# fema-ffrd/gpras

Hardware: AMD Instinct MI355X
Metric: gp_fits_per_sec (higher is better)
Workload: dtype f64; 1 GPU; BASELINE configs[1] as the many-independent-cells workload: exact GP N=4096 d=8 RBF, fit F1 = kernel build + blocked fp64-MFMA Cholesky + alpha + LML, per cell; cells = y columns of one training set with per-cell hyperparameters (the reference's per-mode models); n_train=4096, d=8, kernel=RBF, collective=none (one process), launcher=single process

## Files before the change

### gpras_amd/_lib.py

```python

from __future__ import annotations

import ctypes as C
from pathlib import Path

import numpy as np

import os

LIB_PATH = Path(os.environ["GPRX_LIBRARY"]) if os.environ.get("GPRX_LIBRARY") else Path(__file__).resolve().parent / "libgprx.so"

GPRX_OK, GPRX_EINVAL, GPRX_ENOTPD, GPRX_EHIP, GPRX_ENOMEM, GPRX_ESTATE, GPRX_ERCCL, GPRX_ENOCONV = range(8)
UNIQUE_ID_BYTES = 128
TRAIN_VARIANCE, TRAIN_LENGTHSCALE, TRAIN_NOISE, TRAIN_Z = 1, 2, 4, 8
GEMM_C_LOWER, GEMM_A_LOWER, GEMM_A_UPPER, GEMM_B_LOWER, GEMM_B_UPPER = 1, 2, 4, 8, 16
REDUCE_LOGDET_QUAD, REDUCE_COL, REDUCE_ROWSQ_FINAL, REDUCE_ROW = range(4)

DISTANCE_FORMS = {"difference": 0, "expanded": 1}
KERNEL_IDS = {"RBF": 0, "Matern12": 1, "Matern32": 2, "Matern52": 3, "Exponential": 4}


class GprxLibraryError(RuntimeError):
    """libgprx.so is missing or unusable."""

# ... 120 lines not shown
    "gprx_hms_last_error": (C.c_char_p, [_vp]),
    "gprx_api": (C.c_int, [C.c_int, _vp, _i64, _vp, _i64, _i64, _vp]),
    "gprx_spline_eval": (C.c_int, [C.c_int, _vp, C.c_int, _vp, _vp, _i64, _vp]),
    "gprx_ps_create": (C.c_int, [C.c_int, _i64, _vp, _vp, _i64, _vp, _vp, C.c_int, _vp, _vp, C.c_int, _vp, C.POINTER(_vp)]),
    "gprx_ps_destroy": (C.c_int, [_vp]),
    "gprx_ps_last_error": (C.c_char_p, [_vp]),
    "gprx_ps_set_weights": (C.c_int, [_vp, _vp]),
    "gprx_ps_fit_centerline": (C.c_int, [_vp, _vp, _vp, _vp, _vp, _vp, _i64, _vp]),
    "gprx_ps_timings": (C.c_int, [_vp, _dp]),
    "gprx_ps_rating": (C.c_int, [_vp, _vp, _vp, _i64, _vp, _vp]),
    "gprx_ps_set_boundaries": (C.c_int, [_vp, _vp, _vp, _i64]),
    "gprx_ps_centerline": (C.c_int, [_vp, _vp]),
    "gprx_ps_gather": (C.c_int, [_vp, _vp, _i64, _vp]),
    "gprx_ps_surface": (C.c_int, [_vp, _vp, _vp]),
    "gprx_ps_surface_dev": (C.c_int, [_vp, _i64, _i64, _vp, _i64, _vp, _i64]),
    "gprx_ps_synchronize": (C.c_int, [_vp]),
    "gprx_pca_slab_rows": (C.c_int, [_vp, C.POINTER(_i64)]),
    "gprx_rs_create": (C.c_int, [C.c_int, _i64, _i64, C.c_int, _vp, _vp, _vp, C.POINTER(_vp)]),
    "gprx_rs_destroy": (C.c_int, [_vp]),
    "gprx_rs_last_error": (C.c_char_p, [_vp]),
    "gprx_rs_apply": (C.c_int, [_vp, _vp, _vp, _i64, _vp]),
    "gprx_rs_apply_dev": (C.c_int, [_vp, _i64, _vp, _i64, _vp, _vp, _i64]),
    "gprx_rs_synchronize": (C.c_int, [_vp]),
    "gprx_rs_timings": (C.c_int, [_vp, _dp]),
    "gprx_al_create": (C.c_int, [C.c_int, C.POINTER(_vp)]),
    "gprx_al_destroy": (C.c_int, [_vp]),
    "gprx_al_last_error": (C.c_char_p, [_vp]),
    "gprx_al_synchronize": (C.c_int, [_vp]),
    "gprx_al_cutoff_dev": (C.c_int, [_vp, C.c_int, _vp, _vp, _vp, _i64, C.c_double, C.POINTER(_i64), C.POINTER(_i64), C.POINTER(_i64), _vp]),
    "gprx_al_cutoff": (C.c_int, [_vp, _vp, _i64, _i64, C.c_double, C.POINTER(_i64), C.POINTER(_i64), C.POINTER(_i64), _vp]),
    "gprx_al_clip_dev": (C.c_int, [_vp, _vp, _i64, _i64, _i64, _i64, _vp, _i64]),
    "gprx_al_timings": (C.c_int, [_vp, _dp]),
    "gprx_dg_create": (C.c_int, [C.c_int, C.POINTER(_vp)]),
    "gprx_dg_destroy": (C.c_int, [_vp]),
    "gprx_dg_last_error": (C.c_char_p, [_vp]),
    "gprx_dg_synchronize": (C.c_int, [_vp]),
    "gprx_dg_sort_u64_dev": (C.c_int, [_vp, _vp, _i64, _vp]),
    "gprx_dg_sort_abs_residual_dev": (C.c_int, [_vp, _vp, _vp, _i64, _vp]),
    "gprx_dg_sort_info": (C.c_int, [_vp, _ip, _dp]),
    "gprx_dg_gather_dev": (C.c_int, [_vp, _vp, _i64, _vp, _i64, _vp]),
    "gprx_dg_scatter_summary_dev": (C.c_int, [_vp, _vp, _vp, _i64, _vp]),
    "gprx_dg_detect_dev": (C.c_int, [_vp, _vp, _vp, _i64, _i64, _vp, _vp, _i64, C.c_double, C.c_int, _vp, C.POINTER(_i64)]),
    "gprx_ev_create": (C.c_int, [C.c_int, _i64, _i64, _i64, _vp, _vp, _vp, _vp, _vp, C.POINTER(_vp)]),
    "gprx_ev_create_empty": (C.c_int, [C.c_int, C.POINTER(_vp)]),
    "gprx_ev_destroy": (C.c_int, [_vp]),
    "gprx_ev_last_error": (C.c_char_p, [_vp]),
    "gprx_ev_synchronize": (C.c_int, [_vp]),
    "gprx_ev_maxima": (C.c_int, [_vp, _vp, _vp, _vp]),
    "gprx_ev_return_periods": (C.c_int, [_vp, _i64, _vp, _vp, _vp]),
    "gprx_ev_rp_eval": (C.c_int, [_vp, C.c_int, _vp, _i64, _vp]),
    "gprx_ev_cov": (C.c_int, [_vp, C.c_int, _vp, _vp]),
    "gprx_ev_eigh": (C.c_int, [_vp, _vp, _vp, _ip]),
    "gprx_ev_scores": (C.c_int, [_vp, C.c_int, C.c_int, _vp]),
    "gprx_ev_standardise": (C.c_int, [_vp, _vp]),
    "gprx_ev_farthest": (C.c_int, [_vp, _vp, _i64, C.c_int, _vp, _i64, _i64, _vp, _vp]),
    "gprx_ev_timings": (C.c_int, [_vp, _dp]),
    "gprx_metrics": (C.c_int, [C.c_int, _vp, _vp, _vp, _i64, _i64, C.c_int, C.c_double, _vp, _vp, _vp, C.POINTER(C.c_uint64)]),
    "gprx_metrics_dev": (C.c_int, [C.c_int, _vp, _vp, _vp, _i64, _i64, C.c_int, C.c_double, _vp, _vp, _vp, C.POINTER(C.c_uint64)]),
    "gprx_kmeans_pp": (C.c_int, [C.c_int, _vp, _i64, C.c_int, _vp, C.c_int, C.c_int, _i64, _vp, _vp]),
    "gprx_kmeans_lloyd": (C.c_int, [C.c_int, _vp, _i64, C.c_int, _vp, C.c_int, C.c_double, C.c_int, _vp, _ip, _ip]),
    "gprx_gather_rows": (C.c_int, [C.c_int, _vp, _i64, _i64, _vp, _vp]),
    "gprx_kmat": (C.c_int, [C.c_int, C.c_int, _vp, _i64, _vp, _i64, C.c_int, _vp, C.c_double, C.c_double, _vp, _i64, _i64, _i64, C.c_int]),
    "gprx_gemm": (C.c_int, [C.c_int, C.c_int, C.c_int, _i64, _i64, _i64, C.c_double, _vp, _i64, _vp, _i64, C.c_double, _vp, _i64, C.c_int, C.c_int]),
    "gprx_potrf": (C.c_int, [C.c_int, _vp, _i64, _i64, _i64, _vp, _ip]),
    "gprx_gemm_batched": (C.c_int, [C.c_int, C.c_int, C.c_int, _i64, _i64, _i64, C.c_double, _vp, _i64, _vp, _i64, C.c_double, _vp, _i64, C.c_int, C.c_int,
                                    C.c_int, _i64, _i64, _i64, C.c_int, _i64, _i64, _i64, _vp, C.c_int, _vp, _i64]),
    "gprx_gemm_splitk": (C.c_int, [C.c_int, C.c_int, C.c_int, _i64, _i64, _i64, C.c_double, _vp, _i64, _vp, _i64, C.c_double, _vp, _i64, _vp, C.c_int,
                                   C.c_int, _i64, _i64, _i64, _i64, _vp, C.c_int]),
    "gprx_trsv_lower": (C.c_int, [C.c_int, _vp, _i64, _vp, _vp, _i64, C.c_int, C.c_int, _i64, _vp]),
    "gprx_potrf_batched": (C.c_int, [C.c_int, _vp, _i64, _i64, _i64, _vp, _vp, _vp, C.c_int, _i64, C.c_int, C.c_int, C.c_int, C.c_int, C.c_int, _ip]),
    "gprx_trsm_lower_left": (C.c_int, [C.c_int, _vp, _i64, _vp, _vp, _i64, _i64, _i64, C.c_int, _i64, _vp]),
    "gprx_trtri_lower": (C.c_int, [C.c_int, _vp, _i64, _vp, _vp, _i64, _vp, _i64, _i64, C.c_int, _i64, _i64, C.c_int]),
    "gprx_transpose_inplace": (C.c_int, [C.c_int, _vp, _i64, _i64, C.c_int, _i64]),
    "gprx_alpha_from_inverse": (C.c_int, [C.c_int, _vp, _i64, _vp, _vp, _vp, _i64, C.c_int, _i64, _i64, _i64]),
    "gprx_reduce_probe": (C.c_int, [C.c_int, C.c_int, _vp, _i64, _vp, _i64, _i64, C.c_double, C.c_double, C.c_int, _vp, C.c_int, _vp, C.c_int, _i64, _i64,
                                    _i64, _i64, _vp, _vp, C.c_int]),
    "gprx_set_tuning": (C.c_int, [C.c_char_p, C.c_int]),
    "gprx_set_handle_tuning": (C.c_int, [_vp, C.c_char_p, C.c_int]),
    "gprx_mfma_f64_peak": (C.c_int, [C.c_int, _dp]),
    "gprx_exp_probe": (C.c_int, [C.c_int, C.c_int, _vp, _i64, _vp]),
}

TUNING_KEYS = (
    "outer_block", "update_tile", "no_lookahead", "split_panel", "dag", "rhs_vector", "rows_pair", "cell_kernel", "poison_workspace", "predict_path",
    "sgpr_fused", "sgpr_resident", "wait_handover_us", "sgpr_groups_from", "loeo_blocked_potrf",
    "held_general",
    "pcafit_rowsplit",
)
PCAFIT_ROUTES = ("gram", "covariance")

_lib = None


def load():
    global _lib
    if _lib is not None:
        return _lib
    if not LIB_PATH.exists():
        raise GprxLibraryError(
            f"{LIB_PATH} not found: build it with `python -c 'import __graft_entry__ as g; g.build()'` "
            "(hipcc --offload-arch=gfx950).  gpras_amd has no CPU fallback."
        )
    try:
        lib = C.CDLL(str(LIB_PATH))
    except OSError as exc:
        raise GprxLibraryError(f"cannot load {LIB_PATH}: {exc}") from exc
    for name, (res, args) in PROTOTYPES.items():
        try:
            fn = getattr(lib, name)
        except AttributeError as exc:
            raise GprxLibraryError(f"{LIB_PATH} does not export {name}") from exc
        fn.restype = res
        fn.argtypes = args
    _lib = lib
    return lib


def last_error(handle=None) -> str:
    msg = load().gprx_last_error(handle)
    return msg.decode() if msg else ""


def check(rc: int, handle=None) -> None:
    if rc == GPRX_OK:
        return
    msg = last_error(handle)
    if rc == GPRX_EINVAL:
        raise ValueError(msg)
    if rc == GPRX_ENOTPD:
        raise np.linalg.LinAlgError(msg)
    if rc == GPRX_ENOCONV:
        raise np.linalg.LinAlgError(msg)
    if rc == GPRX_ENOMEM:
        raise MemoryError(msg)
    raise RuntimeError(f"libgprx error {rc}: {msg}")


def as_f64(a) -> np.ndarray:
    return np.ascontiguousarray(a, dtype=np.float64)


def ptr(a: np.ndarray):
    return _vp(a.ctypes.data)


class DeviceBuffer:

    def __init__(self, nbytes: int, device: int = 0):
        self.device = device
        self.nbytes = int(nbytes)
        p = _vp()
        check(load().gprx_dev_malloc(device, self.nbytes, C.byref(p)))
        self.ptr = p

    @classmethod
    def from_array(cls, a, device: int = 0) -> "DeviceBuffer":
        a = as_f64(a)
        buf = cls(a.nbytes, device)
        check(load().gprx_memcpy_h2d(device, buf.ptr, ptr(a), a.nbytes))
        return buf

    def to_array(self, shape) -> np.ndarray:
        out = np.empty(shape, dtype=np.float64)
        assert out.nbytes <= self.nbytes
        check(load().gprx_memcpy_d2h(self.device, ptr(out), self.ptr, out.nbytes))
        return out

# ... 14 lines not shown
```

### gpras_amd/csrc/gprx.hip

```cpp
#include "abi_common.h"

#include <algorithm>
#include <chrono>
#include <cmath>
#include <cstdio>
#include <cstdlib>
#include <cstring>
#include <limits>
#include <map>
#include <mutex>
#include <string>
#include <thread>
#include <vector>

#include "gemm_f64.h"
#include "gprx_common.h"
#include "grad.h"
#include "kmat.h"
#include "potrf.h"
#include "potrf_cell.h"
#include "potrf_dag.h"
#include "sgpr.h"
#include "sgpr_asm.h"
#include "sgpr_fused.h"
// ... 593 lines not shown

int gprx_gemm_splitk(int device, int ta, int tb, int64_t m, int64_t n, int64_t k, double alpha, const double* a_dev, int64_t lda,
                     const double* b_dev, int64_t ldb, double beta, double* c_dev, int64_t ldc, double* ws_dev, int kchunk, int cells,
                     int64_t cell_a, int64_t cell_b, int64_t cell_c, int64_t ws_cell, const double* alpha_tab_dev, int alpha_stride) {
  return guarded(nullptr, [&]() -> int {
    if (const char* why = gemm_probe_invalid(ta, tb, m, n, k, a_dev, lda, b_dev, ldb, c_dev, ldc)) return fail(nullptr, GPRX_EINVAL, why);
    if (!ws_dev || off16(ws_dev)) return fail(nullptr, GPRX_EINVAL, "workspace must be given, 16-byte aligned");
    if (kchunk <= 0 || kchunk % GEMM_BK) return fail(nullptr, GPRX_EINVAL, "kchunk must be a positive multiple of 16");
    if (cells < 1 || alpha_stride < 0) return fail(nullptr, GPRX_EINVAL, "cells must be positive");
    if (odd(cell_a) || odd(cell_b) || odd(cell_c) || odd(ws_cell) || cell_a < 0 || cell_b < 0 || cell_c < 0)
      return fail(nullptr, GPRX_EINVAL, "cell strides must be even");
    if (cells > 1 && ws_cell < (k + kchunk - 1) / kchunk * m * n) return fail(nullptr, GPRX_EINVAL, "ws_cell shorter than the slabs of one cell");
    HIPCHK(nullptr, hipSetDevice(device));
    HIPCHK(nullptr, launch_gemm_splitk(util_stream(), ta, tb, (int)m, (int)n, (int)k, alpha, a_dev, lda, b_dev, ldb, beta, c_dev, ldc, ws_dev, kchunk,
                                       cells, cell_a, cell_b, cell_c, ws_cell, alpha_tab_dev, alpha_stride));
    HIPCHK(nullptr, hipStreamSynchronize(util_stream()));
    return GPRX_OK;
  });
}

int gprx_trsv_lower(int device, const double* l_dev, int64_t lda, const double* inv_diag_dev, double* b_dev, int64_t np, int transpose,
                    int batch, int64_t cs, double* work_dev) {
  return guarded(nullptr, [&]() -> int {
    if (const char* why = solve_probe_invalid(l_dev, lda, inv_diag_dev, np, batch, cs)) return fail(nullptr, GPRX_EINVAL, why);
    if (!b_dev || (work_dev && (!transpose || batch != 1))) return fail(nullptr, GPRX_EINVAL, "work is for the transposed solve of one system");
    HIPCHK(nullptr, hipSetDevice(device));
    HIPCHK(nullptr, trsv_lower(util_stream(), l_dev, lda, inv_diag_dev, b_dev, (int)np, transpose != 0, batch, cs, work_dev));
    HIPCHK(nullptr, hipStreamSynchronize(util_stream()));
    return GPRX_OK;
  });
}

int gprx_trsm_lower_left(int device, const double* l_dev, int64_t lda, const double* inv_diag_dev, double* b_dev, int64_t ldb, int64_t n,
                         int64_t ncols, int cells, int64_t cs, const double* src_dev) {
  return guarded(nullptr, [&]() -> int {
    if (const char* why = solve_probe_invalid(l_dev, lda, inv_diag_dev, n, cells, cs)) return fail(nullptr, GPRX_EINVAL, why);
    if (!b_dev || off16(b_dev) || (src_dev && off16(src_dev))) return fail(nullptr, GPRX_EINVAL, "right-hand side must be given, 16-byte aligned");
    if (ncols <= 0 || ncols > (1 << 30) || ldb < ncols || odd(ldb)) return fail(nullptr, GPRX_EINVAL, "ldb must be even and at least ncols");
    if (src_dev && n != NB) return fail(nullptr, GPRX_EINVAL, "src is for n == 64 only");
    HIPCHK(nullptr, hipSetDevice(device));
    HIPCHK(nullptr, trsm_lower_left(util_stream(), l_dev, lda, inv_diag_dev, b_dev, ldb, (int)n, (int)ncols, cells, cs, src_dev));
    HIPCHK(nullptr, hipStreamSynchronize(util_stream()));
    return GPRX_OK;
  });
}

int gprx_trtri_lower(int device, const double* l_dev, int64_t lda, const double* inv_diag_dev, double* x_dev, int64_t ldx, double* t_dev,
                     int64_t ldt, int64_t np, int cells, int64_t cs_l, int64_t cs_x, int tile) {
  return guarded(nullptr, [&]() -> int {
    if (const char* why = solve_probe_invalid(l_dev, lda, inv_diag_dev, np, cells, cs_l)) return fail(nullptr, GPRX_EINVAL, why);
    if (!x_dev || !t_dev || off16(x_dev) || off16(t_dev)) return fail(nullptr, GPRX_EINVAL, "X and T must be given, 16-byte aligned");
    if (ldx < np || ldt < np || odd(ldx) || odd(ldt) || odd(cs_x) || cs_x < 0) return fail(nullptr, GPRX_EINVAL, "ldx, ldt, cs_x must be even, rows at least np");
    if (tile != 0 && tile != 64 && tile != 128) return fail(nullptr, GPRX_EINVAL, "tile must be 0, 64 or 128");
    HIPCHK(nullptr, hipSetDevice(device));
    HIPCHK(nullptr, trtri_lower(util_stream(), l_dev, lda, inv_diag_dev, x_dev, ldx, t_dev, ldt, (int)np, cells, cs_l, cs_x, tile));
    HIPCHK(nullptr, hipStreamSynchronize(util_stream()));
    return GPRX_OK;
  });
}

int gprx_potrf_batched(int device, double* a_dev, int64_t lda, int64_t np, int64_t extra, double* inv_diag_dev, double* stage_dev,
                       double* yvec_dev, int batch, int64_t cs, int route, int outer_block, int update_tile, int lookahead, int col_base,
                       int* info_host) {
  return guarded(nullptr, [&]() -> int {
    if (!a_dev || !inv_diag_dev || !stage_dev || !info_host) return fail(nullptr, GPRX_EINVAL, "null argument");
    if (np <= 0 || np % NB) return fail(nullptr, GPRX_EINVAL, "np must be a positive multiple of 64");
    if (extra < 0 || np > (1 << 30) || extra > (1 << 30)) return fail(nullptr, GPRX_EINVAL, "extra must not be negative, np and extra at most 2^30");
    if (lda < np || odd(lda) || odd(cs) || cs < 0) return fail(nullptr, GPRX_EINVAL, "lda and cs must be even, lda at least np");
    if (batch > 1 && cs < lda * (np + extra)) return fail(nullptr, GPRX_EINVAL, "cs shorter than one cell's matrix: the cells would overlap");
    if (off16(a_dev) || off16(inv_diag_dev) || off16(stage_dev) || (yvec_dev && off16(yvec_dev)))
      return fail(nullptr, GPRX_EINVAL, "operands must be 16-byte aligned");
    if (batch < 1 || route < 0 || route > 2 || col_base < 0) return fail(nullptr, GPRX_EINVAL, "batch must be positive, route 0, 1 or 2");
    if (yvec_dev && (route != 1 || batch == 1 || extra != 0))
      return fail(nullptr, GPRX_EINVAL, "the vector right-hand side is the split panel's, for batched cells without right-hand-side rows");
    if (route == 2 && extra % NB) return fail(nullptr, GPRX_EINVAL, "the cell kernel takes right-hand-side rows in tiles of 64");
    if (lookahead != 0 && (lookahead != 1 || batch > 1 || route == 2)) return fail(nullptr, GPRX_EINVAL, "look-ahead is for one matrix on routes 0 and 1");
    if (outer_block < 0 || outer_block % NB || (update_tile != 0 && update_tile != 64 && update_tile != 128))
      return fail(nullptr, GPRX_EINVAL, "outer_block must be a multiple of 64, update_tile 0, 64 or 128");
    PotrfTuning tune;
    tune.outer_block = outer_block;
    tune.update_tile = update_tile;
    tune.split_panel = route == 1 ? 1 : -1;
    tune.rows_pair = potrf_tuning().rows_pair;
    HIPCHK(nullptr, hipSetDevice(device));
    hipStream_t st = util_stream();
    int* dinfo = nullptr;
    HIPCHK(nullptr, hipMalloc((void**)&dinfo, sizeof(int) * batch));
    hipError_t e = memset_sync(dinfo, 0, sizeof(int) * batch);
    PotrfStreams ps;
    if (e == hipSuccess && lookahead) e = ps.init();
    if (e == hipSuccess)
      e = route == 2 ? potrf_cells(st, a_dev, lda, (int)np, (int)extra, inv_diag_dev, dinfo, batch, cs, 1, col_base)
                     : potrf_lower(st, a_dev, lda, (int)np, (int)extra, inv_diag_dev, dinfo, stage_dev, nullptr, lookahead ? &ps : nullptr, batch, cs, 1,
                                   &tune, col_base, yvec_dev);
    hipError_t e2 = hipStreamSynchronize(st);
    if (ps.aux && e2 == hipSuccess) e2 = hipStreamSynchronize(ps.aux);
    ps.destroy();
    if (e == hipSuccess && e2 == hipSuccess) e2 = copy_sync(info_host, dinfo, sizeof(int) * batch, hipMemcpyDeviceToHost);
    hipFree(dinfo);
    HIPCHK(nullptr, e);
    HIPCHK(nullptr, e2);
    for (int c = 0; c < batch; ++c)
      if (info_host[c]) return fail(nullptr, GPRX_ENOTPD, "matrix not positive definite");
    return GPRX_OK;
  });
}

int gprx_transpose_inplace(int device, double* x_dev, int64_t ld, int64_t n, int cells, int64_t cs) {
  return guarded(nullptr, [&]() -> int {
    if (!x_dev || off16(x_dev)) return fail(nullptr, GPRX_EINVAL, "X must be given, 16-byte aligned");
    if (n <= 0 || n % 64 || n > (1 << 30) || ld < n || odd(ld) || cells < 1 || odd(cs) || cs < 0)
      return fail(nullptr, GPRX_EINVAL, "n must be a positive multiple of 64, ld and cs even");
    HIPCHK(nullptr, hipSetDevice(device));
    HIPCHK(nullptr, transpose_inplace(util_stream(), x_dev, ld, (int)n, cells, cs));
    HIPCHK(nullptr, hipStreamSynchronize(util_stream()));
    return GPRX_OK;
  });
}

int gprx_alpha_from_inverse(int device, const double* x_dev, int64_t ldx, const double* beta_dev, double* part_dev, double* alpha_dev, int64_t np,
                            int cells, int64_t cs_x, int64_t cs_b, int64_t cs_a) {
  return guarded(nullptr, [&]() -> int {
    if (!x_dev || !beta_dev || !part_dev || !alpha_dev) return fail(nullptr, GPRX_EINVAL, "null argument");
    if (np <= 0 || np % NB || np > (1 << 30) || ldx < np || cells < 1 || cs_x < 0 || cs_b < 0 || cs_a < 0)
      return fail(nullptr, GPRX_EINVAL, "np must be a positive multiple of 64");
    HIPCHK(nullptr, hipSetDevice(device));
    HIPCHK(nullptr, alpha_from_inverse(util_stream(), x_dev, ldx, beta_dev, part_dev, alpha_dev, (int)np, cells, cs_x, cs_b, cs_a));
    HIPCHK(nullptr, hipStreamSynchronize(util_stream()));
    return GPRX_OK;
  });
}

int gprx_reduce_probe(int device, int op, const double* m_dev, int64_t ldm, const double* w_dev, int64_t nrows, int64_t ncols, double base,
                      double scale, int accumulate, double* partial_dev, int rows_per_chunk, double* out_dev, int cells, int64_t m_cell,
                      int64_t w_cell, int64_t p_cell, int64_t out_cell, const double* base_tab_dev, const double* base_tab2_dev, int base_stride) {
  return guarded(nullptr, [&]() -> int {
    if (!m_dev || !out_dev) return fail(nullptr, GPRX_EINVAL, "null argument");
    if (nrows <= 0 || ncols <= 0 || nrows > (1 << 30) || ncols > (1 << 30) || cells < 1) return fail(nullptr, GPRX_EINVAL, "sizes must be positive");
    if (m_cell < 0 || w_cell < 0 || p_cell < 0 || out_cell < 0 || base_stride < 0) return fail(nullptr, GPRX_EINVAL, "negative stride");
    hipStream_t st = nullptr;
    switch (op) {
      case GPRX_REDUCE_LOGDET_QUAD:
        if (ldm < nrows || ncols != nrows || out_cell > (1 << 30)) return fail(nullptr, GPRX_EINVAL, "logdet_quad: square matrix, ldm at least its order");
        HIPCHK(nullptr, hipSetDevice(device));
        st = util_stream();
        hipLaunchKernelGGL(logdet_quad_kernel, dim3(cells), dim3(256), 0, st, m_dev, ldm, w_dev, (int)nrows, out_dev, m_cell, (int)out_cell);
        break;
      case GPRX_REDUCE_COL: {
        if (ldm < ncols || !partial_dev || rows_per_chunk < 1) return fail(nullptr, GPRX_EINVAL, "colreduce: partial and rows_per_chunk needed");
        const int nchunks = (int)((nrows + rows_per_chunk - 1) / rows_per_chunk);
        if (cells > 1 && p_cell < (int64_t)nchunks * ncols) return fail(nullptr, GPRX_EINVAL, "colreduce: p_cell shorter than the partial sums of one cell");
        HIPCHK(nullptr, hipSetDevice(device));
        st = util_stream();
        hipLaunchKernelGGL(colreduce_partial, dim3((unsigned)((ncols + 255) / 256), nchunks, cells), dim3(256), 0, st, m_dev, ldm, w_dev, (int)nrows,
                           (int)ncols, rows_per_chunk, partial_dev, m_cell, w_cell, p_cell);
        hipLaunchKernelGGL(colreduce_final, dim3((unsigned)((ncols + 255) / 256), cells), dim3(256), 0, st, (const double*)partial_dev, nchunks,
                           (int)ncols, base, scale, accumulate, out_dev, p_cell, out_cell, base_tab_dev, base_tab2_dev, base_stride);
        break;
      }
      case GPRX_REDUCE_ROWSQ_FINAL:
        if (ldm < nrows || cells != 1) return fail(nullptr, GPRX_EINVAL, "rowsq_final: one cell, ldm at least nrows");
        HIPCHK(nullptr, hipSetDevice(device));
        st = util_stream();
        hipLaunchKernelGGL(rowsq_final_kernel, dim3((unsigned)((nrows + 255) / 256)), dim3(256), 0, st, m_dev, (int)ncols, ldm, (int)nrows, base, out_dev);
        break;
      case GPRX_REDUCE_ROW:
// ... 5 lines not shown
                           out_dev);
        break;
      default:
        return fail(nullptr, GPRX_EINVAL, "unknown reduction");
    }
    HIPCHK(nullptr, hipGetLastError());
    HIPCHK(nullptr, hipStreamSynchronize(st));
    return GPRX_OK;
  });
}

extern "C" int gprx_dag_stamps(gprx_handle h, unsigned long long* out, int max_words, int* T, int* grid) {
  if (!h || !h->dag.stamps) return 0;
  const int n = (int)std::min<size_t>(h->dag.stamp_words, (size_t)max_words);
  hipStreamSynchronize(h->stream);
  copy_sync(out, h->dag.stamps, sizeof(unsigned long long) * n, hipMemcpyDeviceToHost);
  if (T) *T = h->dag.T;
  if (grid) *grid = h->dag.grid;
  return n;
}

#ifdef GPRX_CHAIN_STAMPS
extern "C" int gprx_chain_stamps(unsigned long long* out16) {
  hipMemcpyFromSymbol(out16, HIP_SYMBOL(gprx::g_chain_stamps), sizeof(unsigned long long) * 16);
  return 0;
}
#endif

#ifdef GPRX_PANEL_ACC
int gprx_panel_acc(unsigned long long* out8, int reset) {
  if (reset) {
    unsigned long long z[8] = {0};
    hipMemcpyToSymbol(HIP_SYMBOL(gprx::g_panel_acc), z, sizeof(z));
  }
  hipMemcpyFromSymbol(out8, HIP_SYMBOL(gprx::g_panel_acc), sizeof(unsigned long long) * 8);
  return 0;
}
#endif
#ifdef GPRX_CELL_ACC
int gprx_cell_acc(unsigned long long* out16, int reset) {
  if (reset) {
    unsigned long long z[16] = {0};
    hipMemcpyToSymbol(HIP_SYMBOL(gprx::g_cell_acc), z, sizeof(z));
  }
  hipMemcpyFromSymbol(out16, HIP_SYMBOL(gprx::g_cell_acc), sizeof(unsigned long long) * 16);
  return 0;
}
#endif
int gprx_sf_stamps(gprx_handle h, int enable, unsigned long long* out) {
  return guarded(h, [&]() -> int {
    if (!h) return fail(h, GPRX_EINVAL, "null handle");
    HIPCHK(h, hipSetDevice(h->device));
    HIPCHK(h, hipStreamSynchronize(h->stream));
    if (out && h->sf_stamps) HIPCHK(h, copy_sync(out, h->sf_stamps, sizeof(unsigned long long) * SF_STAMP_WORDS, hipMemcpyDeviceToHost));
    if (enable && !h->sf_stamps) {
      HIPCHK(h, hipMalloc((void**)&h->sf_stamps, sizeof(unsigned long long) * SF_STAMP_WORDS));
      HIPCHK(h, memset_sync(h->sf_stamps, 0, sizeof(unsigned long long) * SF_STAMP_WORDS));
      drop_graphs(h);
    } else if (!enable && h->sf_stamps) {
      HIPCHK(h, hipFree(h->sf_stamps));
      h->sf_stamps = nullptr;
      drop_graphs(h);
    }
    return GPRX_OK;
  });
}
#ifdef GPRX_PANEL_STAMPS
int gprx_panel_stamps(unsigned long long* out64) {
  hipMemcpyFromSymbol(out64, HIP_SYMBOL(gprx::g_panel_stamps), sizeof(unsigned long long) * 64);
  return 0;
}
#endif

namespace {
bool apply_tuning(PotrfTuning& t, int& predict_path, int& fused, int& resident, const std::string& k, int value) {
  if (k == "outer_block" && value >= 0 && value % 128 == 0) t.outer_block = value;
  else if (k == "update_tile" && (value == 0 || value == 64 || value == 128)) t.update_tile = value;
  else if (k == "no_lookahead") t.no_lookahead = value != 0;
  else if (k == "split_panel" && value >= -1 && value <= 1) t.split_panel = value;
  else if (k == "dag" && value >= -1 && value <= 1) t.dag = value;
  else if (k == "rhs_vector" && value >= -1 && value <= 1) t.rhs_vector = value;
  else if (k == "cell_kernel" && value >= -1 && value <= 1) t.cell_kernel = value;
  else if (k == "rows_pair" && value >= 0 && value <= 1) t.rows_pair = value;
  else if (k == "poison_workspace" && value >= 0 && value <= 1) t.poison_workspace = value;
  else if (k == "predict_path" && value >= 0 && value <= 2) predict_path = value;
  else if (k == "sgpr_fused" && value >= 0 && value <= 1) fused = value;
  else if (k == "sgpr_resident" && value >= 0 && value <= 1) resident = value;
  else if (k == "wait_handover_us" && value >= 0) wait_handover_us() = value;
  else if (k == "sgpr_groups_from" && value >= 0) sf_groups_from() = value;
  else if (k == "loeo_blocked_potrf" && value >= -1 && value <= 2) loeo_blocked_potrf_force() = value;
  else if (k == "pcafit_rowsplit" && value >= 0 && value <= 1) pcafit_rowsplit_tuning() = value;
  else return false;
  return true;
}
}

int gprx_set_tuning(const char* key, int value) {
  return guarded(nullptr, [&]() -> int {
    if (!key) return fail(nullptr, GPRX_EINVAL, "null key");
    if (!apply_tuning(potrf_tuning(), predict_path_tuning(), sgpr_fused_tuning(), sgpr_resident_tuning(), key, value)) return fail(nullptr, GPRX_EINVAL, "unknown tuning key or bad value");
    return GPRX_OK;
  });
}

int gprx_set_handle_tuning(gprx_handle h, const char* key, int value) {
  return guarded(h, [&]() -> int {
    if (!h || !key) return fail(h, GPRX_EINVAL, "null argument");
    const int fused_before = h->sgpr_fused;
    if (std::string(key) == "held_general") {
      if (value < 0 || value > 1) return fail(h, GPRX_EINVAL, "unknown tuning key or bad value");
      h->held_general = value;
    } else if (!apply_tuning(h->tune, h->predict_path, h->sgpr_fused, h->sgpr_resident, key, value)) {
      return fail(h, GPRX_EINVAL, "unknown tuning key or bad value");
    }
    if (hipSetDevice(h->device) == hipSuccess && hipStreamSynchronize(h->stream) == hipSuccess) drop_graphs(h);
    if (h->sgpr_fused != fused_before) {
      h->sarena_slots = 0;
      if (h->m != 0) h->factorized = false;
    }
    return GPRX_OK;
  });
}

int gprx_mfma_f64_peak(int device, double* tflops) {
  return guarded(nullptr, [&]() -> int {
    if (!tflops) return fail(nullptr, GPRX_EINVAL, "null argument");
    HIPCHK(nullptr, hipSetDevice(device));
    double* out = nullptr;
    HIPCHK(nullptr, hipMalloc((void**)&out, 64));
    hipEvent_t e0, e1;
    hipEventCreate(&e0);
    hipEventCreate(&e1);
    const int iters = 20000, blocks = 256 * 4;
    hipStream_t us = util_stream();
    hipLaunchKernelGGL(mfma_f64_peak_kernel, dim3(blocks), dim3(256), 0, us, out, 100);
    hipEventRecord(e0, us);
    hipLaunchKernelGGL(mfma_f64_peak_kernel, dim3(blocks), dim3(256), 0, us, out, iters);
    hipEventRecord(e1, us);
    hipError_t e = hipStreamSynchronize(us);
    float ms = 0.f;
    hipEventElapsedTime(&ms, e0, e1);
    hipEventDestroy(e0);
    hipEventDestroy(e1);
    hipFree(out);
    HIPCHK(nullptr, e);
    const double flops = (double)blocks * 4  * iters * 4  * 2048.0;
    *tflops = flops / (ms * 1e-3) / 1e12;
    return GPRX_OK;
  });
}

}
```

### gpras_amd/csrc/potrf.h

```cpp
#pragma once
#include <cstdlib>
#include <utility>
#include <vector>

#include "chain64.h"
#include "gemm_f64.h"
#include "gprx_common.h"

namespace gprx {

#ifdef GPRX_PANEL_ACC
__device__ unsigned long long g_panel_acc[8];
#define PACC_DECL unsigned long long pacc_prev_ = 0;
#define PACC(i)                                                                                                       \
  {                                                                                                                   \
    if ((i) == 5) __builtin_amdgcn_s_waitcnt(0);                                                                      \
    const unsigned long long t_ = __builtin_amdgcn_s_memtime();                                                       \
    if (threadIdx.x == 0 && blockIdx.x == 0 && blockIdx.y == 0 && gridDim.x > 2) {                                    \
      if ((i) > 0) atomicAdd(&g_panel_acc[i], t_ - pacc_prev_);                                                       \
      else atomicAdd(&g_panel_acc[0], 1ull);                                                                          \
    }                                                                                                                 \
    pacc_prev_ = t_;                                                                                                  \
  }
#else
// ... 345 lines not shown
  PSTAMP(5)
  PACC(5)
}

constexpr int ROWS_WG = 64 * RT;
__device__ __forceinline__ void wave_sync_lds() {
  __builtin_amdgcn_fence(__ATOMIC_RELEASE, "wavefront");
  __builtin_amdgcn_wave_barrier();
  __builtin_amdgcn_fence(__ATOMIC_ACQUIRE, "wavefront");
}
template <int P>
__device__ __forceinline__ void rows_step(d4 (&acc)[RT][4], double* __restrict__ sIn, double* __restrict__ sX, int tid, int wave, int g, int r,
                                          const double* __restrict__ gstage) {
  constexpr int C0 = 8 * P;
  constexpr int KT = C0 / 16;
  constexpr int HALF = P & 1;
  constexpr int WROWS = 16 * RT;
  if ((r >> 3) == HALF) {
#pragma unroll
    for (int rt = 0; rt < RT; ++rt)
#pragma unroll
      for (int q = 0; q < 4; ++q) sIn[(WROWS * wave + 16 * rt + g + 4 * q) * PSUB + (r & 7)] = acc[rt][KT][q];
  }
  wave_sync_lds();
  const int srow = WROWS * wave + (tid & 63);
  if ((tid & 63) < WROWS) {
    double x[8];
#pragma unroll
    for (int k = 0; k < 8; ++k) {
      double t = sIn[srow * PSUB + k];
#pragma unroll
      for (int m = 0; m < k; ++m) t = __builtin_fma(-x[m], gstage[(C0 + k) * NB + C0 + m], t);
      x[k] = t * gstage[NB * NB + C0 + k];
    }
#pragma unroll
    for (int k = 0; k < 8; ++k) sX[srow * PSUB + k] = x[k];
  }
  wave_sync_lds();
  if constexpr (C0 + 8 < NB) {
    constexpr int KT0 = (C0 + 8) / 16;
    double fa[RT][2], fb[4][2];
#pragma unroll
    for (int rt = 0; rt < RT; ++rt)
#pragma unroll
      for (int ks = 0; ks < 2; ++ks) fa[rt][ks] = -sX[(WROWS * wave + 16 * rt + r) * PSUB + 4 * ks + g];
#pragma unroll
    for (int kt = KT0; kt < 4; ++kt) {
      const int kk = kt * 16 + r;
#pragma unroll
      for (int ks = 0; ks < 2; ++ks) fb[kt][ks] = (kk >= C0 + 8) ? gstage[kk * NB + C0 + 4 * ks + g] : 0.0;
    }
#pragma unroll
    for (int kt = KT0; kt < 4; ++kt)
#pragma unroll
      for (int rt = 0; rt < RT; ++rt) {
        acc[rt][kt] = __builtin_amdgcn_mfma_f64_16x16x4f64(fa[rt][0], fb[kt][0], acc[rt][kt], 0, 0, 0);
        acc[rt][kt] = __builtin_amdgcn_mfma_f64_16x16x4f64(fa[rt][1], fb[kt][1], acc[rt][kt], 0, 0, 0);
      }
  }
  if ((r >> 3) == HALF) {
#pragma unroll
    for (int rt = 0; rt < RT; ++rt)
#pragma unroll
      for (int q = 0; q < 4; ++q) acc[rt][KT][q] = sX[(WROWS * wave + 16 * rt + g + 4 * q) * PSUB + (r & 7)];
  }
}

__device__ __forceinline__ d2 ld2_l2(__amdgpu_buffer_rsrc_t rs, unsigned voff, unsigned soff) {
  typedef unsigned int u4v __attribute__((ext_vector_type(4)));
  const u4v v = __builtin_amdgcn_raw_buffer_load_b128(rs, voff, soff, 16);
  d2 out;
  __builtin_memcpy(&out, &v, 16);
  return out;
}
template <int M>
__device__ __forceinline__ double lane_xor(double v) {
  int w[2];
  __builtin_memcpy(w, &v, 8);
  w[0] = __builtin_amdgcn_ds_swizzle(w[0], (M << 10) | 0x1f);
  w[1] = __builtin_amdgcn_ds_swizzle(w[1], (M << 10) | 0x1f);
  __builtin_memcpy(&v, w, 8);
  return v;
}
template <bool FUSE_K64, bool YVEC, bool X_L2, bool Y_IN, bool Y_OUT, bool NT_IN = false, bool NT_OUT = false>
__device__ __forceinline__ void rows_pass(double* __restrict__ A21, int64_t lda, int rows_below, int row0, const double* __restrict__ stage,
                                          double* __restrict__ yv, int64_t ycell, int ybeta, int yrows, double* __restrict__ sIn,
                                          double* __restrict__ sX) {
  constexpr int WROWS = 16 * RT;
  const int lane = __lane_id(), wave = __builtin_amdgcn_readfirstlane(threadIdx.x >> 6), tid = 64 * wave + lane, g = lane >> 4, r = lane & 15;
  d4 acc[RT][4];
  {
    const char* wg0 = reinterpret_cast<const char*>(A21 + (int64_t)row0 * lda);
    unsigned rowp[RT][4];
    bool valid[RT][4];
#pragma unroll
    for (int rt = 0; rt < RT; ++rt)
#pragma unroll
      for (int q = 0; q < 4; ++q) {
        const int lrow = WROWS * wave + 16 * rt + g + 4 * q;
        valid[rt][q] = row0 + lrow < rows_below;
        rowp[rt][q] = ((unsigned)(valid[rt][q] ? lrow : 0) * (unsigned)lda + r) * 8u;
      }
    d4 upd[FUSE_K64 ? RT : 1][4];
    if constexpr (FUSE_K64) {
#pragma unroll
      for (int rt = 0; rt < RT; ++rt)
#pragma unroll
        for (int kt = 0; kt < 4; ++kt) upd[rt][kt] = d4{0.0, 0.0, 0.0, 0.0};
      const double* arow[RT];
      [[maybe_unused]] __amdgpu_buffer_rsrc_t xrs;
      [[maybe_unused]] unsigned xoff[RT];
      if constexpr (X_L2) xrs = __builtin_amdgcn_make_buffer_rsrc(A21 + (int64_t)row0 * lda - NB, 0, 0xffffffff, 0x00020000);
#pragma unroll
      for (int rt = 0; rt < RT; ++rt) {
        const int idx = row0 + WROWS * wave + 16 * rt + r;
        arow[rt] = A21 + (int64_t)(idx < rows_below ? idx : 0) * lda - NB + 4 * g;
        if constexpr (X_L2) xoff[rt] = ((unsigned)(idx < rows_below ? idx - row0 : 0) * (unsigned)lda + 4u * g) * 8u;
      }
      const double* brow = A21 - (int64_t)NB * lda + (int64_t)r * lda - NB + 4 * g;
#pragma unroll
      for (int k0 = 0; k0 < NB; k0 += 16) {
        double fa[RT][4], fb[4][4];
#pragma unroll
        for (int rt = 0; rt < RT; ++rt) {
          d2 lo, hi;
          if constexpr (X_L2) {
            lo = ld2_l2(xrs, xoff[rt], 8u * k0);
            hi = ld2_l2(xrs, xoff[rt], 8u * k0 + 16u);
          } else {
            lo = *reinterpret_cast<const d2*>(arow[rt] + k0);
            hi = *reinterpret_cast<const d2*>(arow[rt] + k0 + 2);
          }
          fa[rt][0] = lo.x; fa[rt][1] = lo.y; fa[rt][2] = hi.x; fa[rt][3] = hi.y;
        }
#pragma unroll
        for (int kt = 0; kt < 4; ++kt) {
          const double* bp = brow + (int64_t)(16 * kt) * lda + k0;
          const d2 lo = *reinterpret_cast<const d2*>(bp), hi = *reinterpret_cast<const d2*>(bp + 2);
          fb[kt][0] = lo.x; fb[kt][1] = lo.y; fb[kt][2] = hi.x; fb[kt][3] = hi.y;
        }
#pragma unroll
        for (int j = 0; j < 4; ++j)
#pragma unroll
          for (int rt = 0; rt < RT; ++rt)
#pragma unroll
            for (int kt = 0; kt < 4; ++kt) upd[rt][kt] = __builtin_amdgcn_mfma_f64_16x16x4f64(fa[rt][j], fb[kt][j], upd[rt][kt], 0, 0, 0);
      }
    }
#pragma unroll
    for (int rt = 0; rt < RT; ++rt)
#pragma unroll
      for (int q = 0; q < 4; ++q)
#pragma unroll
        for (int kt = 0; kt < 4; ++kt) {
          const double* src = reinterpret_cast<const double*>(wg0 + rowp[rt][q] + kt * 128);
          acc[rt][kt][q] = NT_IN ? __builtin_nontemporal_load(src) : *src;
        }
    if constexpr (FUSE_K64) {
#pragma unroll
      for (int rt = 0; rt < RT; ++rt)
#pragma unroll
        for (int kt = 0; kt < 4; ++kt)
#pragma unroll
          for (int q = 0; q < 4; ++q) {
            const double v = -1.0 * upd[rt][kt][q];
            acc[rt][kt][q] = __builtin_fma(1.0, acc[rt][kt][q], v);
          }
    }
#pragma unroll
    for (int rt = 0; rt < RT; ++rt)
#pragma unroll
      for (int q = 0; q < 4; ++q)
#pragma unroll
        for (int kt = 0; kt < 4; ++kt) acc[rt][kt][q] = valid[rt][q] ? acc[rt][kt][q] : 0.0;
  }
  rows_step<0>(acc, sIn, sX, tid, wave, g, r, stage);
  rows_step<1>(acc, sIn, sX, tid, wave, g, r, stage);
  rows_step<2>(acc, sIn, sX, tid, wave, g, r, stage);
  rows_step<3>(acc, sIn, sX, tid, wave, g, r, stage);
  rows_step<4>(acc, sIn, sX, tid, wave, g, r, stage);
  rows_step<5>(acc, sIn, sX, tid, wave, g, r, stage);
  double ybj[YVEC ? 4 : 1], yold[YVEC ? RT : 1][4];
  [[maybe_unused]] int yrow0 = row0;
  if constexpr (YVEC) {
    yv += ycell;
    asm volatile("" : "+s"(yrow0));
#pragma unroll
    for (int kt = 0; kt < 4; ++kt) ybj[kt] = yv[ybeta + 16 * kt + r];
#pragma unroll
    for (int rt = 0; rt < RT; ++rt)
#pragma unroll
      for (int q = 0; q < 4; ++q) {
        const int idx = yrow0 + WROWS * wave + 16 * rt + g + 4 * q;
        yold[rt][q] = Y_IN ? sIn[(WROWS * wave + 16 * rt + g + 4 * q) * PSUB + 8] : yv[yrows + (idx < rows_below ? idx : 0)];
      }
  }
  rows_step<6>(acc, sIn, sX, tid, wave, g, r, stage);
  rows_step<7>(acc, sIn, sX, tid, wave, g, r, stage);
#pragma unroll
  for (int rt = 0; rt < RT; ++rt)
#pragma unroll
    for (int q = 0; q < 4; ++q) {
      const int idx = row0 + WROWS * wave + 16 * rt + g + 4 * q;
      if (idx < rows_below) {
        double* dst = A21 + (int64_t)idx * lda + r;
#pragma unroll
        for (int kt = 0; kt < 4; ++kt) {
          if constexpr (NT_OUT) __builtin_nontemporal_store(acc[rt][kt][q], dst + kt * 16);
          else dst[kt * 16] = acc[rt][kt][q];
        }
      }
    }
  if constexpr (YVEC) {
#pragma unroll
    for (int rt = 0; rt < RT; ++rt)
#pragma unroll
      for (int q = 0; q < 4; ++q) {
        double sum = acc[rt][0][q] * ybj[0];
#pragma unroll
        for (int kt = 1; kt < 4; ++kt) sum = __builtin_fma(acc[rt][kt][q], ybj[kt], sum);
        sum += lane_xor<1>(sum);
        sum += lane_xor<2>(sum);
        sum += lane_xor<4>(sum);
        sum += lane_xor<8>(sum);
        const int idx = yrow0 + WROWS * wave + 16 * rt + g + 4 * q;
        if constexpr (Y_OUT) {
          if (r == 0) sIn[(WROWS * wave + 16 * rt + g + 4 * q) * PSUB + 8] = yold[rt][q] - sum;
        } else {
          if (r == 0 && idx < rows_below) yv[yrows + idx] = yold[rt][q] - sum;
        }
      }
  }
}

template <bool FUSE_K64, bool YVEC>
__global__ __launch_bounds__(256, FUSE_K64 ? 3 : 4) void potrf_rows_kernel(double* __restrict__ A21, int64_t lda, int rows_below,
                                                                           const double* __restrict__ stage, int64_t cs, double* __restrict__ yv) {
  __shared__ __attribute__((aligned(16))) double sIn[ROWS_WG * PSUB];
  __shared__ __attribute__((aligned(16))) double sX[ROWS_WG * PSUB];
  const int64_t off = (int64_t)blockIdx.y * cs;
  rows_pass<FUSE_K64, YVEC, false, false, false>(A21 + off, lda, rows_below, blockIdx.x * ROWS_WG, stage + off, yv, off, 0, NB, sIn, sX);
}

template <bool YVEC>
__global__ __launch_bounds__(256, 3) void potrf_rows_pair_kernel(double* __restrict__ A21, int64_t lda, int rows_below,
                                                                 const double* __restrict__ stage, const double* __restrict__ stage2, int64_t cs,
                                                                 double* __restrict__ yv) {
  __shared__ __attribute__((aligned(16))) double sIn[ROWS_WG * PSUB];
  __shared__ __attribute__((aligned(16))) double sX[ROWS_WG * PSUB];
  const int64_t off = (int64_t)blockIdx.y * cs;
  const int row0 = blockIdx.x * ROWS_WG;
  rows_pass<false, YVEC, false, false, true, true, false>(A21 + off, lda, rows_below, row0, stage + off, yv, off, 0, 2 * NB, sIn, sX);
  asm volatile("s_waitcnt vmcnt(0)" ::: "memory");
  wave_sync_lds();
  int row0b = row0;
  asm volatile("" : "+s"(row0b));
  rows_pass<true, YVEC, true, true, false, true, true>(A21 + off + NB, lda, rows_below, row0b, stage2 + off, yv, off, NB, 2 * NB, sIn, sX);
}

constexpr int STAGE_LD = 129;

struct PotrfProfile {
  std::vector<hipEvent_t> pool;
  size_t used = 0;
  std::vector<std::pair<size_t, double>> gemm_marks;
  std::vector<std::pair<size_t, double>> strip_marks;
  std::vector<size_t> panel_marks;
  hipEvent_t next() {
    if (used == pool.size()) {
      hipEvent_t e;
      hipEventCreate(&e);
      pool.push_back(e);
    }
    return pool[used++];
  }
  void reset() {
    used = 0;
    gemm_marks.clear();
    strip_marks.clear();
    panel_marks.clear();
  }
  ~PotrfProfile() {
    for (auto e : pool) hipEventDestroy(e);
  }
};

struct PotrfTuning {
  int outer_block = 0;
  int update_tile = 0;
  int no_lookahead = 0;
  int split_panel = 0;
  int poison_workspace = 0;
  int cell_kernel = 0;
  int rhs_vector = 0;
  int dag = 0;
  int rows_pair = 1;
};
inline PotrfTuning& potrf_tuning() {
  static PotrfTuning t = [] {
    PotrfTuning v;
    if (const char* e = getenv("GPRX_OUTER_BLOCK")) v.outer_block = atoi(e);
    if (const char* e = getenv("GPRX_UPDATE_TILE")) v.update_tile = atoi(e);
    if (const char* e = getenv("GPRX_SPLIT_PANEL")) v.split_panel = atoi(e);
    if (const char* e = getenv("GPRX_DAG")) v.dag = atoi(e);
    if (const char* e = getenv("GPRX_RHS_VECTOR")) v.rhs_vector = atoi(e);
    if (const char* e = getenv("GPRX_CELL_KERNEL")) v.cell_kernel = atoi(e);
    if (const char* e = getenv("GPRX_ROWS_PAIR")) v.rows_pair = atoi(e) != 0;
    return v;
  }();
  return t;
}

struct PotrfStreams {
  hipStream_t aux = nullptr;
  hipEvent_t block_done = nullptr, tail_done = nullptr;
  hipError_t init() {
    hipError_t e = hipStreamCreateWithFlags(&aux, hipStreamNonBlocking);
    if (e != hipSuccess) return e;
    if ((e = hipEventCreateWithFlags(&block_done, hipEventDisableTiming)) != hipSuccess) return e;
    return hipEventCreateWithFlags(&tail_done, hipEventDisableTiming);
  }
  void destroy() {
    if (aux) hipStreamDestroy(aux);
    if (block_done) hipEventDestroy(block_done);
    if (tail_done) hipEventDestroy(tail_done);
    aux = nullptr;
    block_done = tail_done = nullptr;
  }
};

inline bool potrf_split_panel(const PotrfTuning& tune, int batch) { return tune.split_panel ? tune.split_panel > 0 : batch >= 24; }

inline bool potrf_rhs_vector_ok(const PotrfTuning& tune, int batch) { return tune.rhs_vector >= 0 && batch > 1 && potrf_split_panel(tune, batch); }

inline hipError_t potrf_lower(hipStream_t st, double* A, int64_t lda, int np, int extra, double* inv_diag, int* info,
                              double* diag_stage, PotrfProfile* prof = nullptr, PotrfStreams* ps = nullptr, int batch = 1, int64_t cs = 0,
                              int info_stride = 0, const PotrfTuning* tune_in = nullptr, int col_base = 0, double* yvec = nullptr) {
  const double* prev_stage = nullptr;
  double* prev_dst = nullptr;
  auto mark_gemm = [&](hipStream_t s, int ncols_lower, int rows_rect, int ncols, int k, bool strip = false) {
    if (!prof) return;
    const double elems = 0.5 * (double)ncols_lower * (ncols_lower + 1) + (double)rows_rect * ncols;
    (strip ? prof->strip_marks : prof->gemm_marks).push_back({prof->used, 2.0 * k * elems * batch});
    hipEventRecord(prof->next(), s);
  };
  auto mark_end = [&](hipStream_t s) {
    if (prof) hipEventRecord(prof->next(), s);
  };
  const int total_rows = np + extra;
  const PotrfTuning& tune = tune_in ? *tune_in : potrf_tuning();
  if (tune.no_lookahead) ps = nullptr;
  const int ob = tune.outer_block ? tune.outer_block : (np > 4096 ? 512 : 1024);
  const int bulk_tile = tune.update_tile ? tune.update_tile : 64;
  bool tail_pending = false;
  hipError_t err = hipSuccess;
  const bool split_panel = potrf_split_panel(tune, batch);
  if (yvec && !split_panel) return hipErrorInvalidValue;
  const bool rows_pair = split_panel && batch > 1 && tune.rows_pair != 0;
  auto panel = [&](int c, bool fuse = false, int pair = 0) {
    const int rows_below = total_rows - c - NB;
    double* Acc = A + (int64_t)c * lda + c;
    if (prof) {
      prof->panel_marks.push_back(prof->used);
      hipEventRecord(prof->next(), st);
    }
    double* stage_out = diag_stage + (int64_t)c * STAGE_LD;
    double* invd = inv_diag + (int64_t)(c / NB) * NB * NB;
    double* yv = yvec ? yvec + c : nullptr;
    const int own_rows = split_panel ? (pair == 1 ? NB : 0) : rows_below;
    const int nchunks = (own_rows + PANEL_OWN_ROWS - 1) / PANEL_OWN_ROWS;
    const auto diag = fuse ? potrf_panel_kernel<true> : potrf_panel_kernel<false>;
    hipLaunchKernelGGL(diag, dim3(nchunks + 1, batch), dim3(256), 0, st, Acc, lda,
                       own_rows, nchunks, invd, info, col_base + c, stage_out, prev_stage, prev_dst, NB, cs, info_stride, yv, (int)(pair == 2 && yv));
    if (pair == 2) {
      if (rows_below > 0) {
        const auto rows = yv ? potrf_rows_pair_kernel<true> : potrf_rows_pair_kernel<false>;
        hipLaunchKernelGGL(rows, dim3((rows_below + ROWS_WG - 1) / ROWS_WG, batch), dim3(256), 0, st, Acc + (int64_t)NB * lda - NB, lda, rows_below,
                           (const double*)(stage_out - (int64_t)NB * STAGE_LD), (const double*)stage_out, cs, yv ? yv - NB : nullptr);
      }
    } else if (split_panel && rows_below > 0 && pair == 0) {
      const auto rows = fuse ? (yv ? potrf_rows_kernel<true, true> : potrf_rows_kernel<true, false>)
                             : (yv ? potrf_rows_kernel<false, true> : potrf_rows_kernel<false, false>);
      hipLaunchKernelGGL(rows, dim3((rows_below + ROWS_WG - 1) / ROWS_WG, batch), dim3(256), 0, st, Acc + (int64_t)NB * lda, lda, rows_below,
                         (const double*)stage_out, cs, yv);
    }
    prev_stage = stage_out;
    prev_dst = Acc;
    if (prof) hipEventRecord(prof->next(), st);
  };
  auto update = [&](int c0, int k, int c1, int n, int tile) {
    const int rows = total_rows - c1;
    const double* L21 = A + (int64_t)c1 * lda + c0;
    double* A22 = A + (int64_t)c1 * lda + c1;
    mark_gemm(st, n, rows - n, n, k, k <= 128);
    hipError_t e = launch_gemm(st, 0, 1, rows, n, k, -1.0, L21, lda, L21, lda, 1.0, A22, lda, GEMM_C_LOWER, k == NB ? 64 : tile, batch, cs, cs, cs);
    mark_end(st);
    if (e != hipSuccess && err == hipSuccess) err = e;
  };
  auto factor_range = [&](auto&& self, int c0, int w) -> void {
    if (w <= NB) {
      panel(c0);
      return;
    }
    const int h = ((w / NB + 1) / 2) * NB;
    if (h == NB && w - h == NB && rows_pair) {
      panel(c0, false, 1);
      panel(c0 + h, true, 2);
      return;
    }
    self(self, c0, h);
    if (h == NB && w - h == NB) {
      panel(c0 + h, true);
      return;
    }
    update(c0, h, c0 + h, w - h, 64);
    self(self, c0 + h, w - h);
  };
  for (int C = 0; C < np; C += ob) {
    const int w = (np - C < ob) ? np - C : ob;
    factor_range(factor_range, C, w);
    if (err != hipSuccess) return err;
    const int R = C + w;
    if (R >= np) break;
    const int wn = (np - R < ob) ? np - R : ob;
    if (ps && tail_pending) hipStreamWaitEvent(st, ps->tail_done, 0);
    update(C, w, R, wn, batch > 1 ? bulk_tile : 64);
    if (err != hipSuccess) return err;
    if (ps) hipEventRecord(ps->block_done, st);
    const int R2 = R + wn;
    if (R2 < np) {
      hipStream_t ts = ps ? ps->aux : st;
      if (ps) hipStreamWaitEvent(ts, ps->block_done, 0);
      const int rows = total_rows - R2, cols = np - R2;
      const double* Lrow = A + (int64_t)R2 * lda + C;
      mark_gemm(ts, cols, rows - cols, cols, w);
      hipError_t e = launch_gemm(ts, 0, 1, rows, cols, w, -1.0, Lrow, lda, Lrow, lda, 1.0, A + (int64_t)R2 * lda + R2, lda, GEMM_C_LOWER,
                                   bulk_tile, batch, cs, cs, cs);
      mark_end(ts);
      if (e != hipSuccess) return e;
      if (ps) {
        hipEventRecord(ps->tail_done, ts);
        tail_pending = true;
      }
    }
  }
  if (prev_stage) hipLaunchKernelGGL(copy_block_kernel, dim3(batch), dim3(256), 0, st, prev_stage, prev_dst, lda, NB, cs);
  if (ps && tail_pending) hipStreamWaitEvent(st, ps->tail_done, 0);
  return hipGetLastError();
}

}
```

Measured before the change: 2312 fits/s.

## Hand over first-pass panel results through LDS in the paired rows kernel

In the paired rows kernel, the first pass now writes most of its solved 64-column tile into an LDS image (sImg, reusing sIn/sX lines) and keeps the right-hand-side vector in a separate sY array. The second pass reads those tiles from LDS instead of reloading them from L2. Only one k-tile (XIMG_L2_KT) is still read through L2, behind a waitcnt. This is meant to cut global and L2 traffic and the full vmcnt drain between the two passes. The cost is extra LDS per workgroup, which could lower occupancy under launch_bounds(256,3), and more complex swizzled indexing. It is on by default via rows_handover=1.

```diff
diff --git a/gpras_amd/_lib.py b/gpras_amd/_lib.py
--- a/gpras_amd/_lib.py
+++ b/gpras_amd/_lib.py
@@ -226,7 +226,7 @@
 }
 
 TUNING_KEYS = (
-    "outer_block", "update_tile", "no_lookahead", "split_panel", "dag", "rhs_vector", "rows_pair", "cell_kernel", "poison_workspace", "predict_path",
+    "outer_block", "update_tile", "no_lookahead", "split_panel", "dag", "rhs_vector", "rows_pair", "rows_handover", "cell_kernel", "poison_workspace", "predict_path",
     "sgpr_fused", "sgpr_resident", "wait_handover_us", "sgpr_groups_from", "loeo_blocked_potrf",
     "held_general",
     "pcafit_rowsplit",
diff --git a/gpras_amd/csrc/gprx.hip b/gpras_amd/csrc/gprx.hip
--- a/gpras_amd/csrc/gprx.hip
+++ b/gpras_amd/csrc/gprx.hip
@@ -699,6 +699,7 @@
     tune.update_tile = update_tile;
     tune.split_panel = route == 1 ? 1 : -1;
     tune.rows_pair = potrf_tuning().rows_pair;
+    tune.rows_handover = potrf_tuning().rows_handover;
     HIPCHK(nullptr, hipSetDevice(device));
     hipStream_t st = util_stream();
     int* dinfo = nullptr;
@@ -870,6 +871,7 @@
   else if (k == "rhs_vector" && value >= -1 && value <= 1) t.rhs_vector = value;
   else if (k == "cell_kernel" && value >= -1 && value <= 1) t.cell_kernel = value;
   else if (k == "rows_pair" && value >= 0 && value <= 1) t.rows_pair = value;
+  else if (k == "rows_handover" && value >= 0 && value <= 1) t.rows_handover = value;
   else if (k == "poison_workspace" && value >= 0 && value <= 1) t.poison_workspace = value;
   else if (k == "predict_path" && value >= 0 && value <= 2) predict_path = value;
   else if (k == "sgpr_fused" && value >= 0 && value <= 1) fused = value;
diff --git a/gpras_amd/csrc/potrf.h b/gpras_amd/csrc/potrf.h
--- a/gpras_amd/csrc/potrf.h
+++ b/gpras_amd/csrc/potrf.h
@@ -451,10 +451,23 @@
   __builtin_memcpy(&v, w, 8);
   return v;
 }
-template <bool FUSE_K64, bool YVEC, bool X_L2, bool Y_IN, bool Y_OUT, bool NT_IN = false, bool NT_OUT = false>
+#ifndef GPRX_XIMG_L2_KT
+#define GPRX_XIMG_L2_KT 3
+#endif
+constexpr int XIMG_L2_KT = GPRX_XIMG_L2_KT;
+constexpr int XIMG_UNIT = 256;
+constexpr int XIMG_WAVE = 4 * XIMG_UNIT;
+static_assert(16 * RT * PSUB >= XIMG_UNIT && RT == 2, "a wave's lines of sIn / sX hold one unit each");
+__device__ __forceinline__ double* ximg_unit(int rt, int kt, int wave, double* sIn, double* sX, double* sImg) {
+  const int slot = 2 * (kt - (kt > XIMG_L2_KT ? 1 : 0)) + rt;
+  if (slot == 0) return sX + 16 * RT * PSUB * wave;
+  if (slot == 1) return sIn + 16 * RT * PSUB * wave;
+  return sImg + XIMG_WAVE * wave + XIMG_UNIT * (slot - 2);
+}
+template <bool FUSE_K64, bool YVEC, bool X_L2, bool Y_IN, bool Y_OUT, bool NT_IN = false, bool NT_OUT = false, int X_IMG = 0>
 __device__ __forceinline__ void rows_pass(double* __restrict__ A21, int64_t lda, int rows_below, int row0, const double* __restrict__ stage,
                                           double* __restrict__ yv, int64_t ycell, int ybeta, int yrows, double* __restrict__ sIn,
-                                          double* __restrict__ sX) {
+                                          double* __restrict__ sX, double* __restrict__ sImg = nullptr, double* __restrict__ sY = nullptr) {
   constexpr int WROWS = 16 * RT;
   const int lane = __lane_id(), wave = __builtin_amdgcn_readfirstlane(threadIdx.x >> 6), tid = 64 * wave + lane, g = lane >> 4, r = lane & 15;
   d4 acc[RT][4];
@@ -490,10 +503,16 @@
 #pragma unroll
       for (int k0 = 0; k0 < NB; k0 += 16) {
         double fa[RT][4], fb[4][4];
+        if constexpr (X_L2 && X_IMG == 2)
+          if (k0 == 16 * XIMG_L2_KT) asm volatile("s_waitcnt vmcnt(0)" ::: "memory");
 #pragma unroll
         for (int rt = 0; rt < RT; ++rt) {
           d2 lo, hi;
-          if constexpr (X_L2) {
+          if (X_IMG == 2 && k0 != 16 * XIMG_L2_KT) {
+            const double* u = ximg_unit(rt, k0 / 16, wave, sIn, sX, sImg) + 64 * g;
+            lo = *reinterpret_cast<const d2*>(u + ((r ^ (2 * g)) << 1));
+            hi = *reinterpret_cast<const d2*>(u + 32 + ((r ^ (2 * g + 1)) << 1));
+          } else if constexpr (X_L2) {
             lo = ld2_l2(xrs, xoff[rt], 8u * k0);
             hi = ld2_l2(xrs, xoff[rt], 8u * k0 + 16u);
           } else {
@@ -515,6 +534,7 @@
 #pragma unroll
             for (int kt = 0; kt < 4; ++kt) upd[rt][kt] = __builtin_amdgcn_mfma_f64_16x16x4f64(fa[rt][j], fb[kt][j], upd[rt][kt], 0, 0, 0);
       }
+      if constexpr (X_IMG == 2) wave_sync_lds();
     }
 #pragma unroll
     for (int rt = 0; rt < RT; ++rt)
@@ -561,7 +581,7 @@
 #pragma unroll
       for (int q = 0; q < 4; ++q) {
         const int idx = yrow0 + WROWS * wave + 16 * rt + g + 4 * q;
-        yold[rt][q] = Y_IN ? sIn[(WROWS * wave + 16 * rt + g + 4 * q) * PSUB + 8] : yv[yrows + (idx < rows_below ? idx : 0)];
+        yold[rt][q] = Y_IN ? (X_IMG ? sY[WROWS * wave + 16 * rt + g + 4 * q] : sIn[(WROWS * wave + 16 * rt + g + 4 * q) * PSUB + 8]) : yv[yrows + (idx < rows_below ? idx : 0)];
       }
   }
   rows_step<6>(acc, sIn, sX, tid, wave, g, r, stage);
@@ -580,6 +600,19 @@
         }
       }
     }
+  if constexpr (X_IMG == 1) {
+    wave_sync_lds();
+    const int c = r >> 1;
+#pragma unroll
+    for (int rt = 0; rt < RT; ++rt)
+#pragma unroll
+      for (int kt = 0; kt < 4; ++kt) {
+        if (kt == XIMG_L2_KT) continue;
+        double* u = ximg_unit(rt, kt, wave, sIn, sX, sImg) + 32 * c + (r & 1);
+#pragma unroll
+        for (int q = 0; q < 4; ++q) u[((g + 4 * q) ^ c) << 1] = acc[rt][kt][q];
+      }
+  }
   if constexpr (YVEC) {
 #pragma unroll
     for (int rt = 0; rt < RT; ++rt)
@@ -594,7 +627,7 @@
         sum += lane_xor<8>(sum);
         const int idx = yrow0 + WROWS * wave + 16 * rt + g + 4 * q;
         if constexpr (Y_OUT) {
-          if (r == 0) sIn[(WROWS * wave + 16 * rt + g + 4 * q) * PSUB + 8] = yold[rt][q] - sum;
+          if (r == 0) (X_IMG ? sY[WROWS * wave + 16 * rt + g + 4 * q] : sIn[(WROWS * wave + 16 * rt + g + 4 * q) * PSUB + 8]) = yold[rt][q] - sum;
         } else {
           if (r == 0 && idx < rows_below) yv[yrows + idx] = yold[rt][q] - sum;
         }
@@ -611,20 +644,24 @@
   rows_pass<FUSE_K64, YVEC, false, false, false>(A21 + off, lda, rows_below, blockIdx.x * ROWS_WG, stage + off, yv, off, 0, NB, sIn, sX);
 }
 
-template <bool YVEC>
+template <bool YVEC, bool HAND>
 __global__ __launch_bounds__(256, 3) void potrf_rows_pair_kernel(double* __restrict__ A21, int64_t lda, int rows_below,
                                                                  const double* __restrict__ stage, const double* __restrict__ stage2, int64_t cs,
                                                                  double* __restrict__ yv) {
   __shared__ __attribute__((aligned(16))) double sIn[ROWS_WG * PSUB];
   __shared__ __attribute__((aligned(16))) double sX[ROWS_WG * PSUB];
+  __shared__ __attribute__((aligned(16))) double sImg[HAND ? 4 * XIMG_WAVE : 2];
+  __shared__ __attribute__((aligned(16))) double sY[HAND ? ROWS_WG : 2];
   const int64_t off = (int64_t)blockIdx.y * cs;
   const int row0 = blockIdx.x * ROWS_WG;
-  rows_pass<false, YVEC, false, false, true, true, false>(A21 + off, lda, rows_below, row0, stage + off, yv, off, 0, 2 * NB, sIn, sX);
-  asm volatile("s_waitcnt vmcnt(0)" ::: "memory");
+  rows_pass<false, YVEC, false, false, true, true, false, HAND ? 1 : 0>(A21 + off, lda, rows_below, row0, stage + off, yv, off, 0, 2 * NB, sIn, sX,
+                                                                        sImg, sY);
+  if constexpr (!HAND) asm volatile("s_waitcnt vmcnt(0)" ::: "memory");
   wave_sync_lds();
   int row0b = row0;
   asm volatile("" : "+s"(row0b));
-  rows_pass<true, YVEC, true, true, false, true, true>(A21 + off + NB, lda, rows_below, row0b, stage2 + off, yv, off, NB, 2 * NB, sIn, sX);
+  rows_pass<true, YVEC, true, true, false, true, true, HAND ? 2 : 0>(A21 + off + NB, lda, rows_below, row0b, stage2 + off, yv, off, NB, 2 * NB, sIn,
+                                                                     sX, sImg, sY);
 }
 
 constexpr int STAGE_LD = 129;
@@ -664,6 +701,7 @@
   int rhs_vector = 0;
   int dag = 0;
   int rows_pair = 1;
+  int rows_handover = 1;
 };
 inline PotrfTuning& potrf_tuning() {
   static PotrfTuning t = [] {
@@ -675,6 +713,7 @@
     if (const char* e = getenv("GPRX_RHS_VECTOR")) v.rhs_vector = atoi(e);
     if (const char* e = getenv("GPRX_CELL_KERNEL")) v.cell_kernel = atoi(e);
     if (const char* e = getenv("GPRX_ROWS_PAIR")) v.rows_pair = atoi(e) != 0;
+    if (const char* e = getenv("GPRX_ROWS_HANDOVER")) v.rows_handover = atoi(e) != 0;
     return v;
   }();
   return t;
@@ -743,7 +782,8 @@
                        own_rows, nchunks, invd, info, col_base + c, stage_out, prev_stage, prev_dst, NB, cs, info_stride, yv, (int)(pair == 2 && yv));
     if (pair == 2) {
       if (rows_below > 0) {
-        const auto rows = yv ? potrf_rows_pair_kernel<true> : potrf_rows_pair_kernel<false>;
+        const auto rows = tune.rows_handover ? (yv ? potrf_rows_pair_kernel<true, true> : potrf_rows_pair_kernel<false, true>)
+                                             : (yv ? potrf_rows_pair_kernel<true, false> : potrf_rows_pair_kernel<false, false>);
         hipLaunchKernelGGL(rows, dim3((rows_below + ROWS_WG - 1) / ROWS_WG, batch), dim3(256), 0, st, Acc + (int64_t)NB * lda - NB, lda, rows_below,
                            (const double*)(stage_out - (int64_t)NB * STAGE_LD), (const double*)stage_out, cs, yv ? yv - NB : nullptr);
       }
```

After: 2321 fits/s, median of 6. No clear change (+0.4%).
